# geduardo/SPARC

Hardware: AMD Instinct MI355X
Metric: env-steps/sec at batch 65536 (higher is better)
Workload: dtype f32 wire temperature + f64 scalar state

## Files before the change

### sparc_amd/csrc/wedm_common.h

```cpp
#pragma once


#ifndef WEDM_PACKED_DENSE
#define WEDM_PACKED_DENSE true
#endif
#ifndef WEDM_FUSED_DENSE
#define WEDM_FUSED_DENSE false
#endif
#ifndef WEDM_FUSED_MIN_BLOCKS
#define WEDM_FUSED_MIN_BLOCKS 2
#endif
#ifndef WEDM_PACKED_MIN_BLOCKS
#define WEDM_PACKED_MIN_BLOCKS 2
#endif
#ifndef WEDM_STREAM_PAIRED_LOADS
#define WEDM_STREAM_PAIRED_LOADS 1
#endif
#ifndef WEDM_STREAM_DENSE_QUIET
#define WEDM_STREAM_DENSE_QUIET 1
#endif
#ifndef WEDM_STREAM_REGWALK
#define WEDM_STREAM_REGWALK 1
#endif
#ifndef WEDM_PIN_STAGE
#define WEDM_PIN_STAGE 0
#endif
#ifndef WEDM_PREFETCH_N1
#define WEDM_PREFETCH_N1 0
#endif

#define WEDM_MAX_C 160
#define WEDM_MAX_TILES (WEDM_MAX_C / 8 + 1)
struct WalkTable {
    int32_t C;
    int32_t n_tiles;
    uint32_t zj[WEDM_MAX_TILES * 8];
    uint32_t iv[WEDM_MAX_TILES * 8];
    uint32_t kind[WEDM_MAX_TILES];
    uint32_t split[WEDM_MAX_TILES];
    uint32_t chunk_flags[16][4];
    uint32_t kind_n_mask, kind_s_mask;
    uint32_t split_pack[3];
    uint32_t kind_ne_mask, kind_nj_mask;
    uint32_t kind_n1_mask;
};
enum { TILE_N = 0, TILE_B = 1, TILE_S = 2 };

struct KArgs {
    Hot hot;
    Cold cold;
    int32_t num_envs;
    int32_t n_substeps;
    int32_t n_seg_max;
    const WalkTable* walk;
    int32_t trace_next;
    int32_t trace_slot;
    wedm_trace_desc trace;
    unsigned long long* dbg;
    int32_t* pulse;
    const double* envp;
    const double* wmat;
    double* sig;
};

__device__ __forceinline__ ColdRef kernarg_cold() {
    return ColdRef{(ColdPtr)((const WEDM_AS4 char*)__builtin_amdgcn_kernarg_segment_ptr() + offsetof(KArgs, cold))};
}

__device__ __forceinline__ PulseRef kernarg_pulse() {
    return PulseRef{(PulseSlot)((const WEDM_AS4 char*)__builtin_amdgcn_kernarg_segment_ptr() + offsetof(KArgs, pulse))};
}

__device__ __forceinline__ const double* wedm::kernarg_envp() {
    typedef const double* const WEDM_AS4* EnvpSlot;
    EnvpSlot p = (EnvpSlot)((const WEDM_AS4 char*)__builtin_amdgcn_kernarg_segment_ptr() + offsetof(KArgs, envp));
    asm volatile("" : "+s"(p));
    return *p;
}

__device__ __forceinline__ const double* wedm::kernarg_wmat() {
    typedef const double* const WEDM_AS4* WmatSlot;
    WmatSlot p = (WmatSlot)((const WEDM_AS4 char*)__builtin_amdgcn_kernarg_segment_ptr() + offsetof(KArgs, wmat));
    asm volatile("" : "+s"(p));
    return *p;
}

__device__ __forceinline__ SigRef kernarg_sig() {
    return SigRef{(SigSlot)((const WEDM_AS4 char*)__builtin_amdgcn_kernarg_segment_ptr() + offsetof(KArgs, sig))};
}

#include "wedm_lifecycle.h"

#define WEDM_TRACING(k) (TRACE && (k).trace_next < (k).n_substeps)
#define WEDM_TRACE_POINT(k, it, e, s, SCALAR_LANE, CELLS)                                        \
    if (TRACE && (it) == trace_next) {                                                           \
        const wedm_trace_desc& tr = (k).trace;                                                   \
        const int64_t tcol = trace_column(tr, (e));                                              \
        if (tcol >= 0) {                                                                         \
            if (SCALAR_LANE) trace_scalars(tr, tcol, (s), trace_slot, (k).hot.done_value == 0);  \
            if (tr.T) {                                                                          \
                const int64_t tcnt = tr.env_count;                                               \
                float* tT = tr.T + (int64_t)trace_slot * (k).n_seg_max * tcnt + tcol;            \
                CELLS;                                                                           \
            }                                                                                    \
        }                                                                                        \
        trace_next += tr.every;                                                                  \
        trace_slot = (trace_slot + 1 == tr.capacity) ? 0 : trace_slot + 1;                       \
    }

typedef float f4v __attribute__((ext_vector_type(4)));

struct GlobalT {
    float* base;
    int64_t qstride;
    __device__ __forceinline__ float ld(int i) const { return base[(int64_t)(i >> 2) * qstride + (i & 3)]; }
    __device__ __forceinline__ void st(int i, float v) const { base[(int64_t)(i >> 2) * qstride + (i & 3)] = v; }
    __device__ __forceinline__ f4v ldq(int q) const { return *(const f4v*)(base + (int64_t)q * qstride); }
    __device__ __forceinline__ void stq(int q, f4v v) const { *(f4v*)(base + (int64_t)q * qstride) = v; }
};
__device__ __forceinline__ GlobalT global_wire(float* T, int64_t stride, int64_t e) { return GlobalT{T + 4 * e, 4 * stride}; }

template <int L, bool TO_LDS, class Slot>
__device__ __forceinline__ void copy_wire(float* T, int64_t stride, int64_t e0, int num_envs, int n, int tid, float* lds, Slot slot) {
    constexpr int EPB = 256 / L;
    const int qr = tid / EPB, sel = tid % EPB;
    if (e0 + sel >= num_envs) return;
    float* const base = T + 4 * (e0 + sel);
    const int64_t qstride = 4 * stride;
    const int nq = (n + 3) >> 2;
    for (int q = qr; q < nq; q += L) {
        float* const g = base + (int64_t)q * qstride;
        if (TO_LDS) {
            const f4v v = *(const f4v*)g;
#pragma unroll
            for (int k = 0; k < 4; ++k)
                if (4 * q + k < n) lds[slot(4 * q + k) + sel * L] = v[k];
        } else if (4 * q + 3 < n) {
            f4v v;
#pragma unroll
            for (int k = 0; k < 4; ++k) v[k] = lds[slot(4 * q + k) + sel * L];
            *(f4v*)g = v;
        } else {
#pragma unroll
            for (int k = 0; k < 4; ++k)
                if (4 * q + k < n) g[k] = lds[slot(4 * q + k) + sel * L];
        }
    }
}

template <bool F64, class TA>
__device__ __forceinline__ float stencil_pass(const TA& T, const Geom& g, const Coef& c, const Persist& ps, const Hot& hot,
                                              const StencilF64& f64c, float h_base, float h_zone) {
    const float spool = hot.spool, tref = hot.tref, alpha = hot.alpha, tdiel = hot.tdiel;
    (void)tref; (void)alpha; (void)tdiel;
    const int n = g.n_seg;
    T.st(0, spool);
    float tmax = spool;
    if (n <= 1) return tmax;
    float tm1 = spool;
    float tc = T.ld(1);
    for (int i0 = 1; i0 < n; i0 += 8) {
        float nx[8];
#pragma unroll
        for (int u = 0; u < 8; ++u) {
            int idx = i0 + 1 + u;
            nx[u] = idx < n ? T.ld(idx) : 0.0f;
        }
#pragma unroll
        for (int u = 0; u < 8; ++u) {
            int i = i0 + u;
            if (i < n) {
                float tn;
                if (F64) tn = stencil_cell_f64(i, n, tm1, tc, nx[u], g, c, ps, f64c, h_base, h_zone);
                else tn = stencil_cell(i, n, tm1, tc, nx[u], g, c, ps, tref, alpha, tdiel);
                T.st(i, tn);
                tmax = tn > tmax ? tn : tmax;
                tm1 = tc;
                tc = nx[u];
            }
        }
    }
    return tmax;
}

template <uint32_t F, class TA>
__device__ __forceinline__ void run_substeps_h(const KArgs& k, const Hot& hot, const ColdRef cold, const Geom& g, int64_t e,
                                               uint32_t gid, Env& s, const TA& T, Sig& sg) {
    constexpr bool TRACE = (F & F_TRACE) != 0, F64 = (F & F_F64) != 0, PULSE = (F & F_PULSE) != 0;
    constexpr bool MAT = (F & F_MAT) != 0;
    Persist ps;
    init_persist<false, MAT>(hot, cold, e, s, ps);
    const StencilF64 f64c = stencil_f64_consts<F>(cold, e);
    const bool tracing = WEDM_TRACING(k);
    int trace_next = k.trace_next, trace_slot = k.trace_slot;
    (void)trace_next; (void)trace_slot;
    for (int it = 0; it < k.n_substeps; ++it) {
        if (!s.done) {
            const int32_t pk = PULSE ? pulse_kind(s) : 0;
            Coef c = scalar_prelude<F>(hot, cold, g, e, gid, s, ps, true);
            float tmax = s.broken ? s.tmax : stencil_pass<F64>(T, g, c, ps, hot, f64c, s.h_base, s.h_zone);
            env_step_done<F>(hot, cold, e, s, tmax, pk, true, sg);
        } else if (!tracing) {
            break;
        }
        WEDM_TRACE_POINT(k, it, e, s, true,
                         for (int i = 0; i < g.n_seg; ++i) tT[(int64_t)i * tcnt] = T.ld(i));
    }
}

template <uint32_t F, class TA>
__device__ __forceinline__ void run_substeps(const KArgs& k, const ColdRef cold, const Geom& g, int64_t e,
                                             uint32_t gid, Env& s, const TA& T, Sig& sg) {
    run_substeps_h<F, TA>(k, launch_hot<F>(k, cold, e, true), cold, g, e, gid, s, T, sg);
}

__device__ __forceinline__ float fmax_gt(float a, float b) { return __builtin_fmaxf(a, b); }

template <int CTRL>
__device__ __forceinline__ float dpp_lane_perm(float x) {
    return __int_as_float(__builtin_amdgcn_update_dpp(0, __float_as_int(x), CTRL, 0xF, 0xF, false));
}
template <int L>
__device__ __forceinline__ float max_over_env_lanes(float v) {
    static_assert(L == 1 || L == 2 || L == 4 || L == 8 || L == 16, "lanes per environment");
    if (L >= 2) v = fmax_gt(v, dpp_lane_perm<0xB1>(v));
    if (L >= 4) v = fmax_gt(v, dpp_lane_perm<0x4E>(v));
    if (L >= 8) v = fmax_gt(v, dpp_lane_perm<0x141>(v));
    if (L >= 16) v = fmax_gt(v, dpp_lane_perm<0x140>(v));
    return v;
}

#ifdef WEDM_STAMPS
#ifdef WEDM_STAMPS_REAL
#define WEDM_S2_CLOCK "s_memrealtime"
#else
#define WEDM_S2_CLOCK "s_memtime"
#endif
#define WEDM_S2_STAMP_DECL unsigned long long sst[12] = {0, 0, 0, 0, 0, 0, 0, 0, 0, 0, 0, 0}; \
    asm volatile(WEDM_S2_CLOCK " %0\n\ts_waitcnt lgkmcnt(0)" : "=s"(sst[7])::"memory")
#define WEDM_S2_STAMP(i) do { __builtin_amdgcn_sched_barrier(0); \
    asm volatile(WEDM_S2_CLOCK " %0\n\ts_waitcnt lgkmcnt(0)" : "=s"(sst[i])::"memory"); \
    __builtin_amdgcn_sched_barrier(0); } while (0)
#define WEDM_S2_STAMP_VM(i) do { __builtin_amdgcn_sched_barrier(0); \
    asm volatile("s_waitcnt vmcnt(0)\n\t" WEDM_S2_CLOCK " %0\n\ts_waitcnt lgkmcnt(0)" : "=s"(sst[i])::"memory"); \
    __builtin_amdgcn_sched_barrier(0); } while (0)
#define WEDM_S2_STAMP_OUT() do { if (k.dbg && (threadIdx.x & 63) == 0) { \
    unsigned long long* o = k.dbg + ((size_t)blockIdx.x * 4 + (threadIdx.x >> 6)) * 12; \
    for (int q = 0; q < 12; ++q) o[q] = sst[q]; } } while (0)
#else
#define WEDM_S2_STAMP_DECL do { } while (0)
#define WEDM_S2_STAMP(i) do { } while (0)
#define WEDM_S2_STAMP_VM(i) do { } while (0)
#define WEDM_S2_STAMP_OUT() do { } while (0)
#endif

typedef float f2 __attribute__((ext_vector_type(2)));

#define WEDM_STAGE_FENCE() __builtin_amdgcn_sched_barrier(0)
template <class V, bool JOULE, bool PERCELL, int W>
__device__ __forceinline__ void tile_staged(const V (&old)[10], V (&tn)[8], const int o, float k, float tuf,
                                            const V (&conv)[8], float tdiel, float adv, const V (&jfe)[8],
                                            float alpha, float tref) {
    V a[W], e[W], f[W], r[W];
#pragma unroll
    for (int u = 0; u < W; ++u) {
        a[u] = sub_twice(old[o + u], old[o + u + 1]);
        e[u] = old[o + u + 1] - tdiel;
        f[u] = old[o + u] - old[o + u + 1];
        if (JOULE) r[u] = old[o + u + 1] - tref;
    }
    WEDM_STAGE_FENCE();
#pragma unroll
    for (int u = 0; u < W; ++u) {
        e[u] = (PERCELL ? conv[o + u] : conv[0]) * e[u];
        f[u] = adv * f[u];
        if (JOULE) r[u] = alpha * r[u];
#if WEDM_PIN_STAGE
        asm volatile("" : "+v"(e[u]));
#endif
    }
    WEDM_STAGE_FENCE();
#pragma unroll
    for (int u = 0; u < W; ++u) {
        a[u] = a[u] + old[o + u + 2];
        if (JOULE) r[u] = 1.0f + r[u];
    }
    WEDM_STAGE_FENCE();
#pragma unroll
    for (int u = 0; u < W; ++u) {
        a[u] = k * a[u];
        if (JOULE) r[u] = (PERCELL ? jfe[o + u] : jfe[0]) * r[u];
    }
    WEDM_STAGE_FENCE();
    if (JOULE) {
#pragma unroll
        for (int u = 0; u < W; ++u) a[u] = a[u] + r[u];
        WEDM_STAGE_FENCE();
    }
#pragma unroll
    for (int u = 0; u < W; ++u) a[u] = a[u] - e[u];
    WEDM_STAGE_FENCE();
#pragma unroll
    for (int u = 0; u < W; ++u) a[u] = a[u] + f[u];
    WEDM_STAGE_FENCE();
#pragma unroll
    for (int u = 0; u < W; ++u) a[u] = a[u] * tuf;
    WEDM_STAGE_FENCE();
#pragma unroll
    for (int u = 0; u < W; ++u) tn[o + u] = old[o + u + 1] + a[u];
    WEDM_STAGE_FENCE();
}

#ifndef WEDM_STAGE_W
#define WEDM_STAGE_W 4
#endif
#ifndef WEDM_STAGE_W_PACKED
#define WEDM_STAGE_W_PACKED 2
#endif
template <class V, bool JOULE, bool PERCELL>
__device__ __forceinline__ void tile8_staged(const V (&old)[10], V (&tn)[8], float k, float tuf, const V (&conv)[8],
                                             float tdiel, float adv, const V (&jfe)[8], float alpha, float tref) {
    constexpr int W = sizeof(V) == 8 ? WEDM_STAGE_W_PACKED : WEDM_STAGE_W;
#pragma unroll
    for (int o = 0; o < 8; o += W)
        tile_staged<V, JOULE, PERCELL, W>(old, tn, o, k, tuf, conv, tdiel, adv, jfe, alpha, tref);
}

#ifndef WEDM_QUAD_STAGE_W
#define WEDM_QUAD_STAGE_W 2
#endif
template <bool JOULE, bool PERCELL, int W>
__device__ __forceinline__ void quad_stage_group(const f2 (&tm)[4], const f2 (&tc)[4], const f2 (&tp)[4], f2 (&tn)[4], const int o,
                                                 float k, float tuf, const f2 (&conv)[4], float tdiel, float adv,
                                                 const f2 (&jfe)[4], float alpha, float tref) {
    f2 a[W], e[W], f[W], r[W];
#pragma unroll
    for (int u = 0; u < W; ++u) {
        a[u] = sub_twice(tm[o + u], tc[o + u]);
        e[u] = tc[o + u] - tdiel;
        f[u] = tm[o + u] - tc[o + u];
        if (JOULE) r[u] = tc[o + u] - tref;
    }
    WEDM_STAGE_FENCE();
#pragma unroll
    for (int u = 0; u < W; ++u) {
        e[u] = (PERCELL ? conv[o + u] : conv[0]) * e[u];
        f[u] = adv * f[u];
        if (JOULE) r[u] = alpha * r[u];
    }
    WEDM_STAGE_FENCE();
#pragma unroll
    for (int u = 0; u < W; ++u) {
        a[u] = a[u] + tp[o + u];
        if (JOULE) r[u] = 1.0f + r[u];
    }
    WEDM_STAGE_FENCE();
#pragma unroll
    for (int u = 0; u < W; ++u) {
        a[u] = k * a[u];
        if (JOULE) r[u] = (PERCELL ? jfe[o + u] : jfe[0]) * r[u];
    }
    WEDM_STAGE_FENCE();
    if (JOULE) {
#pragma unroll
        for (int u = 0; u < W; ++u) a[u] = a[u] + r[u];
        WEDM_STAGE_FENCE();
    }
#pragma unroll
    for (int u = 0; u < W; ++u) a[u] = a[u] - e[u];
    WEDM_STAGE_FENCE();
#pragma unroll
    for (int u = 0; u < W; ++u) a[u] = a[u] + f[u];
    WEDM_STAGE_FENCE();
#pragma unroll
    for (int u = 0; u < W; ++u) a[u] = a[u] * tuf;
    WEDM_STAGE_FENCE();
#pragma unroll
    for (int u = 0; u < W; ++u) tn[o + u] = tc[o + u] + a[u];
    WEDM_STAGE_FENCE();
}
template <bool JOULE, bool PERCELL, int W = WEDM_QUAD_STAGE_W>
__device__ __forceinline__ void quad_staged(const f2 (&tm)[4], const f2 (&tc)[4], const f2 (&tp)[4], f2 (&tn)[4], float k,
                                            float tuf, const f2 (&conv)[4], float tdiel, float adv, const f2 (&jfe)[4],
                                            float alpha, float tref) {
#pragma unroll
    for (int o = 0; o < 4; o += W)
        quad_stage_group<JOULE, PERCELL, W>(tm, tc, tp, tn, o, k, tuf, conv, tdiel, adv, jfe, alpha, tref);
}

#ifndef WEDM_REGS_F64_FENCE
#define WEDM_REGS_F64_FENCE 1
#endif
template <bool JOULE>
__device__ __forceinline__ float cell_f64(float tm1, float tc, float tp1, double k64, double tuf64, double conv64, double tdiel64,
                                          double adv64, double jfe64, double alpha64, double tref64) {
    const double m = (double)tm1, t = (double)tc;
    float d = (float)(k64 * (__builtin_fma(-2.0, t, m) + (double)tp1));
    if (JOULE) {
        const double rho_T = 1.0 + alpha64 * (t - tref64);
        d = (float)((double)d + jfe64 * rho_T);
    }
    d = (float)((double)d - conv64 * (t - tdiel64));
    d = (float)((double)d + adv64 * (m - t));
    return (float)(t + (double)d * tuf64);
}

template <bool JOULE, bool PERCELL>
__device__ __forceinline__ void quad_f64(const f2 (&tm)[4], const f2 (&tc)[4], const f2 (&tp)[4], f2 (&tn)[4], const Geom& g,
                                         const f2 (&hc)[4], const Persist& ps, const f2 (&jfl)[4], const StencilF64& h, double jf64) {
    double cA = (double)hc[0].x * g.a64, cB = (double)hc[0].y * g.a64;
    double jA = (JOULE && jfl[0].x != 0.0f) ? jf64 : 0.0, jB = (JOULE && jfl[0].y != 0.0f) ? jf64 : 0.0;
#pragma unroll
    for (int u = 0; u < 4; ++u) {
        if (PERCELL && u > 0) {
            cA = (double)hc[u].x * g.a64; cB = (double)hc[u].y * g.a64;
            jA = (JOULE && jfl[u].x != 0.0f) ? jf64 : 0.0; jB = (JOULE && jfl[u].y != 0.0f) ? jf64 : 0.0;
        }
        tn[u].x = cell_f64<JOULE>(tm[u].x, tc[u].x, tp[u].x, g.k64, g.tuf64, cA, h.tdiel, ps.adv64, jA, h.alpha, h.tref);
#if WEDM_REGS_F64_FENCE < 0
        __builtin_amdgcn_sched_barrier(0);
#endif
        tn[u].y = cell_f64<JOULE>(tm[u].y, tc[u].y, tp[u].y, g.k64, g.tuf64, cB, h.tdiel, ps.adv64, jB, h.alpha, h.tref);
#if WEDM_REGS_F64_FENCE < 0
        __builtin_amdgcn_sched_barrier(0);
#elif WEDM_REGS_F64_FENCE > 0
        if ((u + 1) % WEDM_REGS_F64_FENCE == 0) __builtin_amdgcn_sched_barrier(0);
#endif
    }
}

template <bool F64, bool JOULE, bool PERCELL, int SW>
__device__ __forceinline__ void rw_quad(const f2 (&tm)[4], const f2 (&tc)[4], const f2 (&tp)[4], f2 (&tn)[4], const Geom& g,
                                        const f2 (&conv)[4], float tdiel, const Persist& ps, const f2 (&jfe)[4], float alpha,
                                        float tref, const StencilF64& h, const Coef& cf) {
    if (F64) quad_f64<JOULE, PERCELL>(tm, tc, tp, tn, g, conv, ps, jfe, h, cf.jf64);
    else quad_staged<JOULE, PERCELL, SW>(tm, tc, tp, tn, g.k, g.tuf, conv, tdiel, ps.adv, jfe, alpha, tref);
}
template <bool F64>
__device__ __forceinline__ float rw_cell(int i, int n_seg, float tm1, float tc, float tp1, const Geom& g, const Coef& cf,
                                         const Persist& ps, float tref, float alpha, float tdiel, const StencilF64& h,
                                         float h_base, float h_zone) {
    if (F64) return stencil_cell_f64(i, n_seg, tm1, tc, tp1, g, cf, ps, h, h_base, h_zone);
    return stencil_cell(i, n_seg, tm1, tc, tp1, g, cf, ps, tref, alpha, tdiel);
}

#define WEDM_REPORT_FROZEN(cond)                                                      \
    do {                                                                              \
        if (!kFrozenOk && __any(cond)) {                                              \
            int32_t* const seen = cold->frozen_seen;                                  \
            if (seen && (threadIdx.x & 63) == 0) *seen = 1;                           \
        }                                                                             \
    } while (0)

#ifdef WEDM_STAMPS
#define WEDM_STAMP(var)                                                      \
    do {                                                                     \
        __builtin_amdgcn_sched_barrier(0);                                   \
        asm volatile("s_memtime %0\n\ts_waitcnt lgkmcnt(0)" : "=s"(var)::"memory"); \
        __builtin_amdgcn_sched_barrier(0);                                   \
    } while (0)
#define WEDM_STAMP_DECL unsigned long long st0 = 0, st1 = 0, st2 = 0, st3 = 0, st4 = 0, acc0 = 0, acc1 = 0, acc2 = 0, acc3 = 0, tk0 = 0, tk1 = 0, accN = 0, accB = 0, accS = 0, cntN = 0, cntB = 0, cntS = 0
#define WEDM_STAMP_ACC() do { acc0 += st1 - st0; acc1 += st2 - st1; acc2 += st3 - st2; acc3 += st4 - st3; } while (0)
#define WEDM_STAMP_OUT()                                                                         \
    do {                                                                                         \
        if (k.dbg && (threadIdx.x & 63) == 0) {                                                  \
            unsigned long long* o = k.dbg + ((size_t)blockIdx.x * 4 + (threadIdx.x >> 6)) * 4;   \
            o[0] = acc0; o[1] = acc1; o[2] = acc2; o[3] = acc3;                                  \
            unsigned long long* o2 = k.dbg + (size_t)gridDim.x * 16 + ((size_t)blockIdx.x * 4 + (threadIdx.x >> 6)) * 6; \
            o2[0] = accN; o2[1] = accB; o2[2] = accS; o2[3] = cntN; o2[4] = cntB; o2[5] = cntS;  \
        }                                                                                        \
    } while (0)
#else
#define WEDM_STAMP(var) do { } while (0)
#define WEDM_STAMP_DECL do { } while (0)
#define WEDM_STAMP_ACC() do { } while (0)
#define WEDM_STAMP_OUT() do { } while (0)
#endif
```

### sparc_amd/csrc/wedm_k_regs.h

```cpp
#pragma once

struct cv4 {
    f2 v[4];
    __device__ __forceinline__ explicit cv4(f2 x) : v{x, x, x, x} {}
};

__device__ __forceinline__ float max3_raw(float a, float b, float c) {
    float r;
    asm("v_max3_f32 %0, %1, %2, %3" : "=v"(r) : "v"(a), "v"(b), "v"(c));
    return r;
}


#ifndef WEDM_REGS_DENSE
#define WEDM_REGS_DENSE WEDM_PACKED_DENSE
#endif
#ifndef WEDM_REGS_SW2
#define WEDM_REGS_SW2 2
#endif
#ifndef WEDM_REGS_PIN2
#define WEDM_REGS_PIN2 1
#endif
#ifndef WEDM_REGS_PAIR_SPLIT
#define WEDM_REGS_PAIR_SPLIT 1
#endif
template <int L, uint32_t F>
__global__ void __launch_bounds__(256, L) wedm_step_regs(const KArgs k) {
    static_assert((F & ~(F_TRACE | F_F64 | F_PULSE)) == 0, "forms of wedm_step_regs");
    constexpr bool TRACE = (F & F_TRACE) != 0, F64 = (F & F_F64) != 0, PULSE = (F & F_PULSE) != 0;
    constexpr int CELLS = 128;
    constexpr int H = CELLS / (2 * L);
    static_assert(L == 1 || L == 2, "one or two lanes per environment");
    static_assert(H % 8 == 0 && H / 8 <= 16, "whole tiles");
    constexpr int EPB = 256 / L;
    constexpr int SW = L == 1 ? 4 : WEDM_REGS_SW2;
    constexpr bool kF64 = F64;
    const ColdRef cold = kernarg_cold();
    Hot hv = k.hot;
    if (L == 1 || WEDM_REGS_PIN2 == 2) {
        pin_hot_in_vgprs(hv);
    } else if (WEDM_REGS_PIN2 == 1) {
        pin_mechanics_in_vgprs(hv);
        pin_quiet_in_vgprs(hv);
    }
    const int tid = threadIdx.x;
    const int c = tid % L;
    const int64_t e = (int64_t)blockIdx.x * EPB + tid / L;
    const bool live = e < k.num_envs;
    const bool writer = c == 0;
    const WalkTable* __restrict__ wt = k.walk;
    const int n = k.hot.n_seg;
    const int64_t stride = cold->s.stride;
    const int base = c * 2 * H;

    Env s;
    Geom g;
    Persist ps{0.0f, 0.0f, 0.0f, 0};
    load_geom(k.hot, cold, live ? e : 0, g);
    StencilF64 f64c{0.0, 0.0, 0.0};
    if (F64) {
        const wedm_params* pp = cold->p;
        f64c = StencilF64{pp->temp_ref, pp->alpha_rho, pp->dielectric_temperature};
        g.k64 = pp->k_cond; g.tuf64 = pp->tuf; g.a64 = pp->a_surf;
    }
    if (live) load_env(cold, e, s);
    else { s.done = WEDM_DEAD_LANE; s.unwind = 0.0; s.h_base = 0.0f; s.h_zone = 0.0f; }
    const int nq = (n + 3) >> 2;
    float* const Te = cold->s.T + (live ? e : 0) * 4;
    const int q0 = base / 4;
    f2 P[H];
#pragma unroll
    for (int q = 0; q < H / 4; ++q) {
        const f4v a = (q0 + q < nq) ? *(const f4v*)(Te + (int64_t)(q0 + q) * stride * 4) : f4v{0.0f, 0.0f, 0.0f, 0.0f};
        const f4v b = (q0 + H / 4 + q < nq) ? *(const f4v*)(Te + (int64_t)(q0 + H / 4 + q) * stride * 4) : f4v{0.0f, 0.0f, 0.0f, 0.0f};
#pragma unroll
        for (int u = 0; u < 4; ++u) P[4 * q + u] = f2{a[u], b[u]};
    }
    const float spool = k.hot.spool, tref = k.hot.tref, alpha = k.hot.alpha, tdiel = k.hot.tdiel;
    const bool reinit = live && s.done && WEDM_AUTORESET(cold);
    if (reinit) {
        reinit_env(cold, e, s, writer);
        pulse_reinit<PULSE>(kernarg_pulse(), cold, e, writer);
    }
    if (__any(reinit)) {
#pragma unroll
        for (int m = 0; m < H; ++m) P[m] = reinit ? f2{spool, spool} : P[m];
    }
    if (c == 0) P[0].x = spool;
    unfreeze_wire(k.hot, s);
    const bool frozen0 = s.done;
    if (!s.done) {
        s.ipk = peak_current(cold, s.mode, e);
        init_persist(k.hot, cold, e, s, ps);
    }
    const uint32_t gid = k.hot.env_id_offset + (uint32_t)e;

    const int n_tiles = wt->n_tiles;
    uint32_t zoneA = 0u, zoneB = 0u, jouleA = 0u, jouleB = 0u, joule_any = 0u;
    for (int t = 0; t < n_tiles; ++t) {
        const uint32_t lo = wt->zj[8 * t];
        zoneA |= ((lo >> (2 * c)) & 1u) << t;       zoneB |= ((lo >> (2 * c + 1)) & 1u) << t;
        jouleA |= ((lo >> (16 + 2 * c)) & 1u) << t; jouleB |= ((lo >> (17 + 2 * c)) & 1u) << t;
        joule_any |= ((lo >> 16) != 0u ? 1u : 0u) << t;
    }
    if (L == 1) {
        zoneA = __builtin_amdgcn_readfirstlane(zoneA); zoneB = __builtin_amdgcn_readfirstlane(zoneB);
        jouleA = __builtin_amdgcn_readfirstlane(jouleA); jouleB = __builtin_amdgcn_readfirstlane(jouleB);
    }
    joule_any = __builtin_amdgcn_readfirstlane(joule_any);
    const uint32_t kind_n = __builtin_amdgcn_readfirstlane(wt->kind_n_mask);
    const uint32_t kind_ne = __builtin_amdgcn_readfirstlane(wt->kind_ne_mask), kind_nj = __builtin_amdgcn_readfirstlane(wt->kind_nj_mask);
    const int last_base = (2 * L - 1) * H;
    const uint32_t last_tile = (n > last_base) ? (1u << ((n - 1 - last_base) >> 3)) : 0u;
    const bool owns_last = c == L - 1;

    f2 convp[H / 8];
    auto build_conv = [&]() {
        const float cz = F64 ? s.h_zone : ps.conv_zone, cb = F64 ? s.h_base : ps.conv_base;
#pragma unroll
        for (int t = 0; t < H / 8; ++t)
            convp[t] = f2{((zoneA >> t) & 1u) ? cz : cb, ((zoneB >> t) & 1u) ? cz : cb};
    };
    build_conv();
    const bool tracing = WEDM_TRACING(k);
    int trace_next = k.trace_next, trace_slot = k.trace_slot;
    (void)trace_next; (void)trace_slot;

    for (int it = 0; it < k.n_substeps; ++it) {
        if (__all(s.done) && !tracing) break;
        const int32_t pk = PULSE ? pulse_kind(s) : 0;
        Coef cf{0.0f, 0.0f, 0, -1};
        QuietTry qt;
        const bool was_quiet = quiet_prelude_t<WEDM_REGS_DENSE, 0u, L == 2 && WEDM_REGS_PAIR_SPLIT>(hv, cold, g, e, gid, s, qt, cf);
        if (!was_quiet) {
            if (!s.done) cf = scalar_prelude(hv, cold, g, e, gid, s, ps, writer, qt);
            build_conv();
        }
        freeze_wire(s);
        const bool act = !s.done;
        float tmax = spool;
        if (L == 1) asm volatile("" : "+s"(zoneA), "+s"(zoneB), "+s"(jouleA), "+s"(jouleB));
        else asm volatile("" : "+v"(zoneA), "+v"(zoneB), "+v"(jouleA), "+v"(jouleB));
        Geom gw = g;
        gw.n_seg = __builtin_amdgcn_readfirstlane(g.n_seg); gw.az_start = __builtin_amdgcn_readfirstlane(g.az_start);
        gw.az_end = __builtin_amdgcn_readfirstlane(g.az_end); gw.cb = __builtin_amdgcn_readfirstlane(g.cb);
        gw.ct = __builtin_amdgcn_readfirstlane(g.ct);
        asm volatile("" : "+s"(gw.n_seg), "+s"(gw.az_start), "+s"(gw.az_end), "+s"(gw.cb), "+s"(gw.ct));
        int nw = __builtin_amdgcn_readfirstlane(n);
        asm volatile("" : "+s"(nw));
        const float a_last = P[H - 1].x, b_first = P[0].y;
        float halo_l = spool, halo_r = 0.0f;
        if (L == 2) {
            const float give = c == 0 ? P[H - 1].y : P[0].x;
            const float got = __int_as_float(swap_with_neighbour(__float_as_int(give)));
            halo_l = c == 0 ? spool : got;
            halo_r = c == 0 ? got : 0.0f;
        }
        const float rw_h_base = s.h_base, rw_h_zone = s.h_zone;
#include "wedm_regs_walk.inc"
        if (L == 2) tmax = fmax_gt(tmax, __int_as_float(swap_with_neighbour(__float_as_int(tmax))));
        unfreeze_wire(hv, s);
        if (!s.done) {
            scalar_epilogue(hv, s, tmax);
            pulse_tally<PULSE>(kernarg_pulse(), cold, e, s, pk, writer);
            if (s.ctrl) control_step_outputs(cold, e, s, writer);
        }
        WEDM_TRACE_POINT(k, it, e, s, writer,
                         float* pa = tT + (int64_t)base * tcnt; float* pb = pa + (int64_t)H * tcnt;
                         int na = n - base; int nb = na - H;
                         asm volatile("" : "+v"(na), "+v"(nb));
                         _Pragma("unroll") for (int m = 0; m < H; ++m) {
                             if (m < na) *pa = P[m].x;
                             if (m < nb) *pb = P[m].y;
                             pa += tcnt; pb += tcnt;
                             asm volatile("" : "+v"(pa), "+v"(pb));
                         });
    }

    if (live) {
#pragma unroll
        for (int q = 0; q < 2 * H / 4; ++q) {
            const int m = (q % (H / 4)) * 4;
            const bool hi = q >= H / 4;
            const f4v w = hi ? f4v{P[m].y, P[m + 1].y, P[m + 2].y, P[m + 3].y} : f4v{P[m].x, P[m + 1].x, P[m + 2].x, P[m + 3].x};
            const int cell = base + 4 * q;
            if (cell + 3 < n) {
                *(f4v*)(Te + (int64_t)(q0 + q) * stride * 4) = w;
            } else {
#pragma unroll
                for (int u = 0; u < 4; ++u)
                    if (cell + u < n) Te[(int64_t)(q0 + q) * stride * 4 + u] = w[u];
            }
        }
    }
    if (live && writer) {
        if (WEDM_REWARD_ON(cold)) {
            if (!frozen0) write_reward(cold, e, s);
            else cold->s.reward[e] = 0.0f;
        }
        store_time_hi(cold, e, s, (uint32_t)k.n_substeps * (uint32_t)k.hot.dt_us);
        store_env(cold, e, s);
    }
}


__device__ __forceinline__ float dpp_row_shr1(float old, float x) {
    return __int_as_float(__builtin_amdgcn_update_dpp(__float_as_int(old), __float_as_int(x), 0x111, 0xF, 0xF, false));
}
__device__ __forceinline__ float dpp_row_shl1(float old, float x) {
    return __int_as_float(__builtin_amdgcn_update_dpp(__float_as_int(old), __float_as_int(x), 0x101, 0xF, 0xF, false));
}
template <int CTRL>
__device__ __forceinline__ float dpp_perm(float x) {
    return __int_as_float(__builtin_amdgcn_update_dpp(0, __float_as_int(x), CTRL, 0xF, 0xF, false));
}

#ifndef WEDM_WIDE_MIN_BLOCKS
#define WEDM_WIDE_MIN_BLOCKS 1
#endif

#ifndef WEDM_WIDE_SW
#define WEDM_WIDE_SW 2
#endif
#ifndef WEDM_WIDE_DENSE
#define WEDM_WIDE_DENSE WEDM_REGS_DENSE
#endif
#ifndef WEDM_WIDE_AUTO_MAX_LANES
#define WEDM_WIDE_AUTO_MAX_LANES 65536
#endif
constexpr int wide_min_blocks(uint32_t F) { return !(F & F_F64) ? WEDM_WIDE_MIN_BLOCKS : (F & F_MINB2) ? 2 : 1; }
template <int L, uint32_t F>
__global__ void __launch_bounds__(256, wide_min_blocks(F)) wedm_step_regs_wide(const KArgs k) {
    static_assert((F & ~(F_CUT | F_TRACE | F_F64 | F_MINB2 | F_PULSE)) == 0 && (!(F & F_MINB2) || (F & F_F64)),
                  "forms of wedm_step_regs_wide");
    constexpr bool CUT = (F & F_CUT) != 0, TRACE = (F & F_TRACE) != 0, F64 = (F & F_F64) != 0, PULSE = (F & F_PULSE) != 0;
    constexpr int H = 16, MINB = wide_min_blocks(F);
    static_assert(H % 8 == 0 && H <= 32, "whole tiles");
    static_assert(L == 4 || L == 8 || L == 16, "the lanes of an environment lie in one DPP row");
    constexpr int EPB = 256 / L;
    constexpr int SW = WEDM_WIDE_SW;
    const ColdRef cold = kernarg_cold();
    Hot hv = k.hot;
    if (MINB == 1) pin_hot_in_vgprs(hv);
    const int tid = threadIdx.x;
    const int c = tid % L;
    const int64_t e = (int64_t)blockIdx.x * EPB + tid / L;
    const bool live = e < k.num_envs;
    const bool writer = c == 0;
    const int n = k.hot.n_seg;
    const int64_t stride = cold->s.stride;
    const int base = c * 2 * H;

    Env s;
    Geom g;
    Persist ps{0.0f, 0.0f, 0.0f, 0};
    load_geom(k.hot, cold, live ? e : 0, g);
    StencilF64 f64c{0.0, 0.0, 0.0};
    if (F64) {
        const wedm_params* pp = cold->p;
        f64c = StencilF64{pp->temp_ref, pp->alpha_rho, pp->dielectric_temperature};
        g.k64 = pp->k_cond; g.tuf64 = pp->tuf; g.a64 = pp->a_surf;
    }
    if (live) load_env(cold, e, s);
    else { s.done = WEDM_DEAD_LANE; s.unwind = 0.0; s.h_base = 0.0f; s.h_zone = 0.0f; }
    const int nq = (n + 3) >> 2;
    float* const Te = cold->s.T + (live ? e : 0) * 4;
    const int q0 = base / 4;
    f2 P[H];
#pragma unroll
    for (int q = 0; q < H / 4; ++q) {
        const f4v a = (q0 + q < nq) ? *(const f4v*)(Te + (int64_t)(q0 + q) * stride * 4) : f4v{0.0f, 0.0f, 0.0f, 0.0f};
        const f4v b = (q0 + H / 4 + q < nq) ? *(const f4v*)(Te + (int64_t)(q0 + H / 4 + q) * stride * 4) : f4v{0.0f, 0.0f, 0.0f, 0.0f};
#pragma unroll
        for (int u = 0; u < 4; ++u) P[4 * q + u] = f2{a[u], b[u]};
    }
    const float spool = k.hot.spool, tref = k.hot.tref, alpha = k.hot.alpha, tdiel = k.hot.tdiel;
    const bool reinit = live && s.done && WEDM_AUTORESET(cold);
    if (reinit) {
        reinit_env(cold, e, s, writer);
        pulse_reinit<PULSE>(kernarg_pulse(), cold, e, writer);
    }
    if (__any(reinit)) {
#pragma unroll
        for (int m = 0; m < H; ++m) P[m] = reinit ? f2{spool, spool} : P[m];
    }
    if (c == 0) P[0].x = spool;
    unfreeze_wire(k.hot, s);
    const bool frozen0 = s.done;
    if (!s.done) {
        s.ipk = peak_current(cold, s.mode, e);
        init_persist(k.hot, cold, e, s, ps);
    }
    const uint32_t gid = k.hot.env_id_offset + (uint32_t)e;

    const int nA = min(max(n - base, 0), H), nB = min(max(n - base - H, 0), H);
    uint32_t zoneA = 0u, zoneB = 0u, jouleA = 0u, jouleB = 0u;
#pragma unroll
    for (int m = 0; m < H; ++m) {
        const int ia = base + m, ib = base + H + m;
        zoneA |= (ia >= g.az_start && ia < g.az_end) ? (1u << m) : 0u;
        zoneB |= (ib >= g.az_start && ib < g.az_end) ? (1u << m) : 0u;
        jouleA |= (ia >= g.cb && ia <= g.ct) ? (1u << m) : 0u;
        jouleB |= (ib >= g.cb && ib <= g.ct) ? (1u << m) : 0u;
    }
    uint32_t cut = 0u;
    if (CUT) {
#pragma unroll
        for (int t = 0; t < H / 8; ++t)
            cut |= __any((nA > 8 * t && nA < 8 * t + 8) || (nB > 8 * t && nB < 8 * t + 8)) ? (1u << t) : 0u;
        cut = __builtin_amdgcn_readfirstlane(cut);
    }
    const int ll = n - 1 - base;
    const bool owns_last = ll >= 0 && ll < 2 * H;
    const int lloc = (n - 1) & (2 * H - 1);
    const bool last_in_b = lloc >= H;
    const uint32_t last_tile = ((n & 7) == 0) ? (1u << ((lloc & (H - 1)) >> 3)) : 0u;
    f2 jm[H], convc[H];
#pragma unroll
    for (int m = 0; m < H; ++m) jm[m] = f2{((jouleA >> m) & 1u) ? 1.0f : 0.0f, ((jouleB >> m) & 1u) ? 1.0f : 0.0f};
    auto build_conv = [&]() {
        const float cz = F64 ? s.h_zone : ps.conv_zone, cb = F64 ? s.h_base : ps.conv_base;
#pragma unroll
        for (int m = 0; m < H; ++m)
            convc[m] = f2{((zoneA >> m) & 1u) ? cz : cb, ((zoneB >> m) & 1u) ? cz : cb};
    };
    build_conv();
    WEDM_STAMP_DECL;
    const bool tracing = WEDM_TRACING(k);
    int trace_next = k.trace_next, trace_slot = k.trace_slot;
    (void)trace_next; (void)trace_slot;

    for (int it = 0; it < k.n_substeps; ++it) {
        if (__all(s.done) && !tracing) break;
        WEDM_STAMP(st0);
        const int32_t pk = PULSE ? pulse_kind(s) : 0;
        Coef cf{0.0f, 0.0f, 0, -1};
        QuietTry qt;
        const bool was_quiet = quiet_prelude_t<WEDM_WIDE_DENSE>(hv, cold, g, e, gid, s, qt, cf);
        if (!was_quiet) {
            if (!s.done) cf = scalar_prelude(hv, cold, g, e, gid, s, ps, writer, qt);
            build_conv();
        }
        freeze_wire(s);
        WEDM_STAMP(st1);
        const bool act = !s.done;
        float tmax = spool;
        const float a_last = P[H - 1].x, b_first = P[0].y;
        float halo_l = dpp_row_shr1(spool, P[H - 1].y), halo_r = dpp_row_shl1(0.0f, P[0].x);
        if (L < 16) { halo_l = c == 0 ? spool : halo_l; halo_r = c == L - 1 ? 0.0f : halo_r; }
        const bool busy = __any(cf.joule_on != 0 || cf.pidx >= 0 || cf.q != 0.0f);
        auto walk = [&](auto plain_tag) {
            constexpr bool PLAIN = decltype(plain_tag)::value;
            const Coef cz{0.0f, 0.0f, 0, -1};
            const Coef& cw = PLAIN ? cz : cf;
            Geom gw = g;
            int nw = n;
            auto prep_gw = [&]() {
                gw.n_seg = __builtin_amdgcn_readfirstlane(g.n_seg); gw.az_start = __builtin_amdgcn_readfirstlane(g.az_start);
                gw.az_end = __builtin_amdgcn_readfirstlane(g.az_end); gw.cb = __builtin_amdgcn_readfirstlane(g.cb);
                gw.ct = __builtin_amdgcn_readfirstlane(g.ct);
                asm volatile("" : "+s"(gw.n_seg), "+s"(gw.az_start), "+s"(gw.az_end), "+s"(gw.cb), "+s"(gw.ct));
                nw = __builtin_amdgcn_readfirstlane(n);
                asm volatile("" : "+s"(nw));
            };
            if (!PLAIN) prep_gw();
            const float jf_lane = (!PLAIN && cf.joule_on) ? (F64 ? 1.0f : cf.jf) : 0.0f;
            const bool joule_wave = !PLAIN && __any(jf_lane != 0.0f);
            const int pcell = (!PLAIN && cf.pidx >= 1 && cf.pidx >= base && cf.pidx < base + 2 * H) ? cf.pidx - base : -1;
            uint32_t ptiles = 0u;
            if (!PLAIN && __any(pcell >= 0)) {
                const int pt = pcell >= 0 ? ((pcell & (H - 1)) >> 3) : -1;
#pragma unroll
                for (int t = 0; t < H / 8; ++t) ptiles |= __any(pt == t) ? (1u << t) : 0u;
            }
            const uint32_t odd = ptiles | last_tile | cut;
            const f2 jfp = f2{jf_lane, jf_lane};
            f2 leftp = f2{halo_l, a_last};
#pragma unroll
            for (int t = 0; t < H / 8; ++t) {
                const int j = 8 * t;
                f2 tm[8], tc[8], tp[8], pn[8];
#pragma unroll
                for (int u = 0; u < 8; ++u) {
                    tc[u] = P[j + u];
                    tm[u] = u == 0 ? leftp : P[j + u - 1];
                    tp[u] = (j + u + 1 < H) ? P[j + u + 1 < H ? j + u + 1 : 0] : f2{b_first, halo_r};
                }
                leftp = tc[7];
                {
                    f2 tmA[4], tcA[4], tpA[4], pnA[4], tmB[4], tcB[4], tpB[4], pnB[4], cvA[4], cvB[4];
#pragma unroll
                    for (int u = 0; u < 4; ++u) {
                        tmA[u] = tm[u]; tcA[u] = tc[u]; tpA[u] = tp[u]; tmB[u] = tm[4 + u]; tcB[u] = tc[4 + u]; tpB[u] = tp[4 + u];
                        cvA[u] = convc[j + u]; cvB[u] = convc[j + 4 + u];
                    }
                    if (!PLAIN && joule_wave) {
                        f2 jvA[4], jvB[4];
#pragma unroll
                        for (int u = 0; u < 4; ++u) { jvA[u] = jm[j + u] * jfp; jvB[u] = jm[j + 4 + u] * jfp; }
                        rw_quad<F64, true, true, SW>(tmA, tcA, tpA, pnA, g, cvA, tdiel, ps, jvA, alpha, tref, f64c, cf);
                        rw_quad<F64, true, true, SW>(tmB, tcB, tpB, pnB, g, cvB, tdiel, ps, jvB, alpha, tref, f64c, cf);
                    } else {
                        rw_quad<F64, false, true, SW>(tmA, tcA, tpA, pnA, g, cvA, tdiel, ps, cvA, alpha, tref, f64c, cw);
                        rw_quad<F64, false, true, SW>(tmB, tcB, tpB, pnB, g, cvB, tdiel, ps, cvB, alpha, tref, f64c, cw);
                    }
#pragma unroll
                    for (int u = 0; u < 4; ++u) { pn[u] = pnA[u]; pn[4 + u] = pnB[u]; }
                    if (t == 0) pn[0].x = (c == 0) ? spool : pn[0].x;
                    if ((odd >> t) & 1u) {
                        if (PLAIN) prep_gw();
                        if ((last_tile >> t) & 1u) {
                            const float x = rw_cell<F64>(base + (last_in_b ? H : 0) + j + 7, nw, last_in_b ? tm[7].y : tm[7].x,
                                                         last_in_b ? tc[7].y : tc[7].x, 0.0f, gw, cw, ps, tref, alpha, tdiel, f64c, s.h_base, s.h_zone);
                            const bool hx = owns_last && !last_in_b, hy = owns_last && last_in_b;
                            pn[7].x = hx ? x : pn[7].x; pn[7].y = hy ? x : pn[7].y;
                        }
                        if ((cut >> t) & 1u) {
                            int lw = lloc;
                            asm volatile("" : "+s"(lw));
#pragma unroll
                            for (int u = 0; u < 8; ++u) {
                                if (lw == j + u) {
                                    const float x = rw_cell<F64>(base + j + u, nw, tm[u].x, tc[u].x, 0.0f, gw, cw, ps, tref, alpha, tdiel, f64c, s.h_base, s.h_zone);
                                    pn[u].x = owns_last ? x : pn[u].x;
                                }
                                if (lw == H + j + u) {
                                    const float x = rw_cell<F64>(base + H + j + u, nw, tm[u].y, tc[u].y, 0.0f, gw, cw, ps, tref, alpha, tdiel, f64c, s.h_base, s.h_zone);
                                    pn[u].y = owns_last ? x : pn[u].y;
                                }
                            }
                        }
                        if (!PLAIN && ((ptiles >> t) & 1u)) {
#pragma unroll
                            for (int u = 0; u < 8; ++u) {
                                if (__any(pcell == j + u)) {
                                    const float x = rw_cell<F64>(base + j + u, nw, (base + j + u == 1) ? spool : tm[u].x, tc[u].x, tp[u].x, gw, cf, ps, tref, alpha, tdiel, f64c, s.h_base, s.h_zone);
                                    pn[u].x = (pcell == j + u) ? x : pn[u].x;
                                }
                                if (__any(pcell == H + j + u)) {
                                    const float x = rw_cell<F64>(base + H + j + u, nw, tm[u].y, tc[u].y, tp[u].y, gw, cf, ps, tref, alpha, tdiel, f64c, s.h_base, s.h_zone);
                                    pn[u].y = (pcell == H + j + u) ? x : pn[u].y;
                                }
                            }
                        }
                    }
                    float mx, my;
                    if ((cut >> t) & 1u) {
                        mx = spool; my = spool;
                        int va = nA, vb = nB;
                        asm volatile("" : "+v"(va), "+v"(vb));
#pragma unroll
                        for (int u = 0; u < 8; ++u) {
                            mx = (j + u < va) ? fmax_gt(mx, pn[u].x) : mx;
                            my = (j + u < vb) ? fmax_gt(my, pn[u].y) : my;
                        }
                    } else {
                        mx = max3_raw(pn[0].x, pn[1].x, pn[2].x); my = max3_raw(pn[0].y, pn[1].y, pn[2].y);
                        mx = max3_raw(mx, pn[3].x, pn[4].x); my = max3_raw(my, pn[3].y, pn[4].y);
                        mx = max3_raw(mx, pn[5].x, pn[6].x); my = max3_raw(my, pn[5].y, pn[6].y);
                        mx = fmax_gt(mx, pn[7].x); my = fmax_gt(my, pn[7].y);
                        mx = nA > j ? mx : spool; my = nB > j ? my : spool;
                    }
                    tmax = max3_raw(tmax, mx, my);
                }
#pragma unroll
                for (int u = 0; u < 8; ++u) P[j + u] = pn[u];
            }
        };
        if (act) {
            if (busy) walk(std::false_type{});
            else walk(std::true_type{});
        }
        WEDM_STAMP(st2);
        tmax = fmax_gt(tmax, dpp_perm<0xB1>(tmax));
        tmax = fmax_gt(tmax, dpp_perm<0x4E>(tmax));
        if (L >= 8) tmax = fmax_gt(tmax, dpp_perm<0x141>(tmax));
        if (L >= 16) tmax = fmax_gt(tmax, dpp_perm<0x140>(tmax));
        unfreeze_wire(hv, s);
        WEDM_STAMP(st3);
        if (!s.done) {
            scalar_epilogue(hv, s, tmax);
            pulse_tally<PULSE>(kernarg_pulse(), cold, e, s, pk, writer);
            if (s.ctrl) control_step_outputs(cold, e, s, writer);
        }
        WEDM_STAMP(st4);
        WEDM_STAMP_ACC();
        WEDM_TRACE_POINT(k, it, e, s, writer,
                         for (int m = 0; m < H; ++m) {
                             if (base + m < n) tT[(int64_t)(base + m) * tcnt] = P[m].x;
                             if (base + H + m < n) tT[(int64_t)(base + H + m) * tcnt] = P[m].y;
                         });
    }
    WEDM_STAMP_OUT();

    if (live) {
#pragma unroll
        for (int q = 0; q < 2 * H / 4; ++q) {
            const int m = (q % (H / 4)) * 4;
            const bool hi = q >= H / 4;
            const f4v w = hi ? f4v{P[m].y, P[m + 1].y, P[m + 2].y, P[m + 3].y} : f4v{P[m].x, P[m + 1].x, P[m + 2].x, P[m + 3].x};
            const int cell = base + 4 * q;
            if (cell + 3 < n) {
                *(f4v*)(Te + (int64_t)(q0 + q) * stride * 4) = w;
            } else {
#pragma unroll
                for (int u = 0; u < 4; ++u)
                    if (cell + u < n) Te[(int64_t)(q0 + q) * stride * 4 + u] = w[u];
            }
        }
    }
    if (live && writer) {
        if (WEDM_REWARD_ON(cold)) {
            if (!frozen0) write_reward(cold, e, s);
            else cold->s.reward[e] = 0.0f;
        }
        store_time_hi(cold, e, s, (uint32_t)k.n_substeps * (uint32_t)k.hot.dt_us);
        store_env(cold, e, s);
    }
}
```

### sparc_amd/csrc/wedm_regs_walk.inc

```
        if (act) {
            const bool all_slow = __any(cf.q < 0.0f);
            const float jf_lane = cf.joule_on ? (kF64 ? 1.0f : cf.jf) : 0.0f;
            const bool joule_wave = __any(jf_lane != 0.0f);
            const uint32_t n_now = all_slow ? 0u : (kind_n | kind_ne | (joule_wave ? 0u : kind_nj));
            const int pcell = (cf.pidx >= 1 && cf.pidx >= base && cf.pidx < base + 2 * H) ? cf.pidx - base : -1;
            uint32_t ptiles = 0u;
            if (__any(pcell >= 0)) {
                const int pt = pcell >= 0 ? ((pcell & (H - 1)) >> 3) : -1;
#pragma unroll
                for (int t = 0; t < H / 8; ++t) ptiles |= __any(pt == t) ? (1u << t) : 0u;
            }
            const uint32_t general = ~n_now | (joule_wave ? joule_any : 0u) | ptiles | last_tile;
            f2 leftp = f2{halo_l, a_last};
#pragma unroll
            for (int t = 0; t < H / 8; ++t) {
                if (t < n_tiles) {
                    const int j = 8 * t;
                    f2 tm[8], tc[8], tp[8], pn[8];
#pragma unroll
                    for (int u = 0; u < 8; ++u) {
                        tc[u] = P[j + u];
                        tm[u] = u == 0 ? leftp : P[j + u - 1];
                        tp[u] = (j + u + 1 < H) ? P[j + u + 1 < H ? j + u + 1 : 0] : f2{b_first, halo_r};
                    }
                    leftp = tc[7];
                    f2 cv[4], jv[4];
                    cv[0] = convp[t];
                    f2 tmA[4], tcA[4], tpA[4], pnA[4], tmB[4], tcB[4], tpB[4], pnB[4];
#pragma unroll
                    for (int u = 0; u < 4; ++u) { tmA[u] = tm[u]; tcA[u] = tc[u]; tpA[u] = tp[u]; tmB[u] = tm[4 + u]; tcB[u] = tc[4 + u]; tpB[u] = tp[4 + u]; }
                    if (!((general >> t) & 1u)) {
                        jv[0] = f2{0.0f, 0.0f};
                        rw_quad<kF64, false, false, SW>(tmA, tcA, tpA, pnA, g, cv, tdiel, ps, jv, alpha, tref, f64c, cf);
                        rw_quad<kF64, false, false, SW>(tmB, tcB, tpB, pnB, g, cv, tdiel, ps, jv, alpha, tref, f64c, cf);
#pragma unroll
                        for (int u = 0; u < 4; ++u) { pn[u] = pnA[u]; pn[4 + u] = pnB[u]; }
                        if (t == 0) pn[0].x = (c == 0) ? spool : pn[0].x;
                        float m0 = max3_raw(tmax, pn[0].x, pn[0].y), m1 = max3_raw(pn[1].x, pn[1].y, pn[2].x);
                        m0 = max3_raw(m0, pn[2].y, pn[3].x); m1 = max3_raw(m1, pn[3].y, pn[4].x);
                        m0 = max3_raw(m0, pn[4].y, pn[5].x); m1 = max3_raw(m1, pn[5].y, pn[6].x);
                        m0 = max3_raw(m0, pn[6].y, pn[7].x);
                        tmax = max3_raw(m0, m1, pn[7].y);
                    } else if (((n_now | (all_slow ? 0u : kind_nj)) >> t) & 1u) {
                        jv[0] = f2{((jouleA >> t) & 1u) ? jf_lane : 0.0f, ((jouleB >> t) & 1u) ? jf_lane : 0.0f};
                        if (!((n_now >> t) & 1u)) {
                            f2 jq[8];
#pragma unroll
                            for (int u = 0; u < 8; ++u) {
                                const uint32_t zj = wt->zj[j + u];
                                jq[u] = f2{((zj >> (16 + 2 * c)) & 1u) ? jf_lane : 0.0f, ((zj >> (17 + 2 * c)) & 1u) ? jf_lane : 0.0f};
                            }
                            f2 jvA[4], jvB[4];
#pragma unroll
                            for (int u = 0; u < 4; ++u) { jvA[u] = jq[u]; jvB[u] = jq[4 + u]; }
                            rw_quad<kF64, true, true, SW>(tmA, tcA, tpA, pnA, g, cv4(cv[0]).v, tdiel, ps, jvA, alpha, tref, f64c, cf);
                            rw_quad<kF64, true, true, SW>(tmB, tcB, tpB, pnB, g, cv4(cv[0]).v, tdiel, ps, jvB, alpha, tref, f64c, cf);
                        } else if (joule_wave && ((joule_any >> t) & 1u)) {
                            rw_quad<kF64, true, false, SW>(tmA, tcA, tpA, pnA, g, cv, tdiel, ps, jv, alpha, tref, f64c, cf);
                            rw_quad<kF64, true, false, SW>(tmB, tcB, tpB, pnB, g, cv, tdiel, ps, jv, alpha, tref, f64c, cf);
                        } else {
                            rw_quad<kF64, false, false, SW>(tmA, tcA, tpA, pnA, g, cv, tdiel, ps, jv, alpha, tref, f64c, cf);
                            rw_quad<kF64, false, false, SW>(tmB, tcB, tpB, pnB, g, cv, tdiel, ps, jv, alpha, tref, f64c, cf);
                        }
#pragma unroll
                        for (int u = 0; u < 4; ++u) { pn[u] = pnA[u]; pn[4 + u] = pnB[u]; }
                        if (t == 0) pn[0].x = (c == 0) ? spool : pn[0].x;
                        const bool has_last = ((last_tile >> t) & 1u) && owns_last;
                        float m0 = max3_raw(tmax, pn[0].x, pn[0].y), m1 = max3_raw(pn[1].x, pn[1].y, pn[2].x);
                        m0 = max3_raw(m0, pn[2].y, pn[3].x); m1 = max3_raw(m1, pn[3].y, pn[4].x);
                        m0 = max3_raw(m0, pn[4].y, pn[5].x); m1 = max3_raw(m1, pn[5].y, pn[6].x);
                        m0 = max3_raw(m0, pn[6].y, pn[7].x);
                        tmax = max3_raw(m0, m1, has_last ? spool : pn[7].y);
                        if ((last_tile >> t) & 1u) {
                            const float x = rw_cell<kF64>(base + H + j + 7, nw, tm[7].y, tc[7].y, 0.0f, gw, cf, ps, tref, alpha, tdiel, f64c, rw_h_base, rw_h_zone);
                            pn[7].y = has_last ? x : pn[7].y;
                            tmax = has_last ? fmax_gt(tmax, x) : tmax;
                        }
                        if ((ptiles >> t) & 1u) {
#pragma unroll
                            for (int u = 0; u < 8; ++u) {
                                if (__any(pcell == j + u)) {
                                    const float x = rw_cell<kF64>(base + j + u, nw, (base + j + u == 1) ? spool : tm[u].x, tc[u].x, tp[u].x, gw, cf, ps, tref, alpha, tdiel, f64c, rw_h_base, rw_h_zone);
                                    pn[u].x = (pcell == j + u) ? x : pn[u].x;
                                    tmax = (pcell == j + u) ? fmax_gt(tmax, x) : tmax;
                                }
                                if (__any(pcell == H + j + u)) {
                                    const float x = rw_cell<kF64>(base + H + j + u, nw, tm[u].y, tc[u].y, tp[u].y, gw, cf, ps, tref, alpha, tdiel, f64c, rw_h_base, rw_h_zone);
                                    pn[u].y = (pcell == H + j + u) ? x : pn[u].y;
                                    tmax = (pcell == H + j + u) ? fmax_gt(tmax, x) : tmax;
                                }
                            }
                        }
                    } else {
#pragma unroll
                        for (int u = 0; u < 8; ++u) {
                            pn[u] = tc[u];
                            const int ia = base + j + u, ib = base + H + j + u;
                            {
                                const float x = (ia >= 1) ? rw_cell<kF64>(ia, nw, (ia == 1) ? spool : tm[u].x, tc[u].x, tp[u].x, gw, cf, ps, tref, alpha, tdiel, f64c, rw_h_base, rw_h_zone) : spool;
                                pn[u].x = ia < nw ? x : pn[u].x;
                                tmax = ia < nw ? fmax_gt(tmax, x) : tmax;
                            }
                            {
                                const float x = rw_cell<kF64>(ib, nw, tm[u].y, tc[u].y, tp[u].y, gw, cf, ps, tref, alpha, tdiel, f64c, rw_h_base, rw_h_zone);
                                pn[u].y = ib < nw ? x : pn[u].y;
                                tmax = ib < nw ? fmax_gt(tmax, x) : tmax;
                            }
                        }
                    }
#pragma unroll
                    for (int u = 0; u < 8; ++u) P[j + u] = pn[u];
#ifdef WEDM_REGS_WALK_TILE_FENCE
                    __builtin_amdgcn_sched_barrier(0);
#endif
                }
            }
        }
```

Baseline: 16.46 billion.

## Pack tile masks, recompute env index, add plain-step fast path in walk

Packs the four per-lane zone/joule tile bitmasks into one 32-bit word and recomputes the environment index from the wave base and lane id instead of keeping it live across the substep loop, both to cut register pressure. The walk also gains a wave-uniform fast path: when no lane in the wave has joule heating, a pulse cell or nonzero charge, it skips the per-lane coefficient checks and uses precomputed scalar tile masks. Optional timing stamps split quiet and non-quiet steps for profiling. The extra packing and unpacking adds ALU work, and the fast-path branch adds a wave vote every substep.

```diff
diff --git a/sparc_amd/csrc/wedm_common.h b/sparc_amd/csrc/wedm_common.h
--- a/sparc_amd/csrc/wedm_common.h
+++ b/sparc_amd/csrc/wedm_common.h
@@ -461,6 +461,11 @@
     } while (0)
 #define WEDM_STAMP_DECL unsigned long long st0 = 0, st1 = 0, st2 = 0, st3 = 0, st4 = 0, acc0 = 0, acc1 = 0, acc2 = 0, acc3 = 0, tk0 = 0, tk1 = 0, accN = 0, accB = 0, accS = 0, cntN = 0, cntB = 0, cntS = 0
 #define WEDM_STAMP_ACC() do { acc0 += st1 - st0; acc1 += st2 - st1; acc2 += st3 - st2; acc3 += st4 - st3; } while (0)
+#define WEDM_STAMP_ACC_SPLIT(quiet)                                                             \
+    do {                                                                                        \
+        if (quiet) { WEDM_STAMP_ACC(); ++cntS; }                                                \
+        else { accN += st1 - st0; accB += st2 - st1; accS += st4 - st2; ++cntN; }               \
+    } while (0)
 #define WEDM_STAMP_OUT()                                                                         \
     do {                                                                                         \
         if (k.dbg && (threadIdx.x & 63) == 0) {                                                  \
@@ -474,5 +479,6 @@
 #define WEDM_STAMP(var) do { } while (0)
 #define WEDM_STAMP_DECL do { } while (0)
 #define WEDM_STAMP_ACC() do { } while (0)
+#define WEDM_STAMP_ACC_SPLIT(quiet) do { } while (0)
 #define WEDM_STAMP_OUT() do { } while (0)
 #endif
diff --git a/sparc_amd/csrc/wedm_k_regs.h b/sparc_amd/csrc/wedm_k_regs.h
--- a/sparc_amd/csrc/wedm_k_regs.h
+++ b/sparc_amd/csrc/wedm_k_regs.h
@@ -45,7 +45,14 @@
     }
     const int tid = threadIdx.x;
     const int c = tid % L;
-    const int64_t e = (int64_t)blockIdx.x * EPB + tid / L;
+    int64_t e = (int64_t)blockIdx.x * EPB + tid / L;
+    const uint32_t wave_env0 = __builtin_amdgcn_readfirstlane((uint32_t)e);
+    auto env_index = [&]() -> int64_t {
+        uint32_t all = ~0u;
+        asm volatile("" : "+s"(all));
+        const uint32_t lane = __builtin_amdgcn_mbcnt_hi(all, __builtin_amdgcn_mbcnt_lo(all, 0u));
+        return (int64_t)(wave_env0 + lane / L);
+    };
     const bool live = e < k.num_envs;
     const bool writer = c == 0;
     const WalkTable* __restrict__ wt = k.walk;
@@ -66,7 +73,7 @@
     if (live) load_env(cold, e, s);
     else { s.done = WEDM_DEAD_LANE; s.unwind = 0.0; s.h_base = 0.0f; s.h_zone = 0.0f; }
     const int nq = (n + 3) >> 2;
-    float* const Te = cold->s.T + (live ? e : 0) * 4;
+    float* Te = cold->s.T + (live ? e : 0) * 4;
     const int q0 = base / 4;
     f2 P[H];
 #pragma unroll
@@ -93,20 +100,17 @@
         s.ipk = peak_current(cold, s.mode, e);
         init_persist(k.hot, cold, e, s, ps);
     }
-    const uint32_t gid = k.hot.env_id_offset + (uint32_t)e;
-
+
+    static_assert(H / 8 <= 8, "tile flags: a byte per mask");
     const int n_tiles = wt->n_tiles;
-    uint32_t zoneA = 0u, zoneB = 0u, jouleA = 0u, jouleB = 0u, joule_any = 0u;
+    uint32_t tile_flags = 0u, joule_any = 0u;
     for (int t = 0; t < n_tiles; ++t) {
         const uint32_t lo = wt->zj[8 * t];
-        zoneA |= ((lo >> (2 * c)) & 1u) << t;       zoneB |= ((lo >> (2 * c + 1)) & 1u) << t;
-        jouleA |= ((lo >> (16 + 2 * c)) & 1u) << t; jouleB |= ((lo >> (17 + 2 * c)) & 1u) << t;
+        tile_flags |= (((lo >> (2 * c)) & 1u) << t) | (((lo >> (2 * c + 1)) & 1u) << (8 + t));
+        tile_flags |= (((lo >> (16 + 2 * c)) & 1u) << (16 + t)) | (((lo >> (17 + 2 * c)) & 1u) << (24 + t));
         joule_any |= ((lo >> 16) != 0u ? 1u : 0u) << t;
     }
-    if (L == 1) {
-        zoneA = __builtin_amdgcn_readfirstlane(zoneA); zoneB = __builtin_amdgcn_readfirstlane(zoneB);
-        jouleA = __builtin_amdgcn_readfirstlane(jouleA); jouleB = __builtin_amdgcn_readfirstlane(jouleB);
-    }
+    if (L == 1) tile_flags = __builtin_amdgcn_readfirstlane(tile_flags);
     joule_any = __builtin_amdgcn_readfirstlane(joule_any);
     const uint32_t kind_n = __builtin_amdgcn_readfirstlane(wt->kind_n_mask);
     const uint32_t kind_ne = __builtin_amdgcn_readfirstlane(wt->kind_ne_mask), kind_nj = __builtin_amdgcn_readfirstlane(wt->kind_nj_mask);
@@ -116,18 +120,23 @@
 
     f2 convp[H / 8];
     auto build_conv = [&]() {
+        const uint32_t zoneA = tile_flags & 0xFFu, zoneB = (tile_flags >> 8) & 0xFFu;
         const float cz = F64 ? s.h_zone : ps.conv_zone, cb = F64 ? s.h_base : ps.conv_base;
 #pragma unroll
         for (int t = 0; t < H / 8; ++t)
             convp[t] = f2{((zoneA >> t) & 1u) ? cz : cb, ((zoneB >> t) & 1u) ? cz : cb};
     };
     build_conv();
+    WEDM_STAMP_DECL;
     const bool tracing = WEDM_TRACING(k);
     int trace_next = k.trace_next, trace_slot = k.trace_slot;
     (void)trace_next; (void)trace_slot;
 
     for (int it = 0; it < k.n_substeps; ++it) {
         if (__all(s.done) && !tracing) break;
+        WEDM_STAMP(st0);
+        e = env_index();
+        const uint32_t gid = k.hot.env_id_offset + (uint32_t)e;
         const int32_t pk = PULSE ? pulse_kind(s) : 0;
         Coef cf{0.0f, 0.0f, 0, -1};
         QuietTry qt;
@@ -137,10 +146,12 @@
             build_conv();
         }
         freeze_wire(s);
+        WEDM_STAMP(st1);
         const bool act = !s.done;
         float tmax = spool;
-        if (L == 1) asm volatile("" : "+s"(zoneA), "+s"(zoneB), "+s"(jouleA), "+s"(jouleB));
-        else asm volatile("" : "+v"(zoneA), "+v"(zoneB), "+v"(jouleA), "+v"(jouleB));
+        if (L == 1) asm volatile("" : "+s"(tile_flags));
+        else asm volatile("" : "+v"(tile_flags));
+        const uint32_t jouleA = (tile_flags >> 16) & 0xFFu, jouleB = tile_flags >> 24;
         Geom gw = g;
         gw.n_seg = __builtin_amdgcn_readfirstlane(g.n_seg); gw.az_start = __builtin_amdgcn_readfirstlane(g.az_start);
         gw.az_end = __builtin_amdgcn_readfirstlane(g.az_end); gw.cb = __builtin_amdgcn_readfirstlane(g.cb);
@@ -158,13 +169,17 @@
         }
         const float rw_h_base = s.h_base, rw_h_zone = s.h_zone;
 #include "wedm_regs_walk.inc"
+        WEDM_STAMP(st2);
         if (L == 2) tmax = fmax_gt(tmax, __int_as_float(swap_with_neighbour(__float_as_int(tmax))));
         unfreeze_wire(hv, s);
+        WEDM_STAMP(st3);
         if (!s.done) {
             scalar_epilogue(hv, s, tmax);
             pulse_tally<PULSE>(kernarg_pulse(), cold, e, s, pk, writer);
             if (s.ctrl) control_step_outputs(cold, e, s, writer);
         }
+        WEDM_STAMP(st4);
+        WEDM_STAMP_ACC_SPLIT(was_quiet);
         WEDM_TRACE_POINT(k, it, e, s, writer,
                          float* pa = tT + (int64_t)base * tcnt; float* pb = pa + (int64_t)H * tcnt;
                          int na = n - base; int nb = na - H;
@@ -176,7 +191,10 @@
                              asm volatile("" : "+v"(pa), "+v"(pb));
                          });
     }
-
+    WEDM_STAMP_OUT();
+
+    e = env_index();
+    Te = cold->s.T + (live ? e : 0) * 4;
     if (live) {
 #pragma unroll
         for (int q = 0; q < 2 * H / 4; ++q) {
diff --git a/sparc_amd/csrc/wedm_regs_walk.inc b/sparc_amd/csrc/wedm_regs_walk.inc
--- a/sparc_amd/csrc/wedm_regs_walk.inc
+++ b/sparc_amd/csrc/wedm_regs_walk.inc
@@ -1,16 +1,27 @@
         if (act) {
-            const bool all_slow = __any(cf.q < 0.0f);
-            const float jf_lane = cf.joule_on ? (kF64 ? 1.0f : cf.jf) : 0.0f;
-            const bool joule_wave = __any(jf_lane != 0.0f);
-            const uint32_t n_now = all_slow ? 0u : (kind_n | kind_ne | (joule_wave ? 0u : kind_nj));
-            const int pcell = (cf.pidx >= 1 && cf.pidx >= base && cf.pidx < base + 2 * H) ? cf.pidx - base : -1;
+            uint32_t n_now = __builtin_amdgcn_readfirstlane(kind_n | kind_ne | kind_nj);
+            uint32_t general = __builtin_amdgcn_readfirstlane(~(kind_n | kind_ne | kind_nj) | last_tile);
+            asm volatile("" : "+s"(n_now), "+s"(general));
+            bool all_slow = false, joule_wave = false;
+            float jf_lane = 0.0f;
+            int pcell = -1;
             uint32_t ptiles = 0u;
-            if (__any(pcell >= 0)) {
-                const int pt = pcell >= 0 ? ((pcell & (H - 1)) >> 3) : -1;
+#ifndef WEDM_REGS_WALK_NO_PLAIN
+            if (__any(cf.joule_on != 0 || cf.pidx >= 0 || cf.q != 0.0f))
+#endif
+            {
+                all_slow = __any(cf.q < 0.0f);
+                jf_lane = cf.joule_on ? (kF64 ? 1.0f : cf.jf) : 0.0f;
+                joule_wave = __any(jf_lane != 0.0f);
+                n_now = all_slow ? 0u : (kind_n | kind_ne | (joule_wave ? 0u : kind_nj));
+                pcell = (cf.pidx >= 1 && cf.pidx >= base && cf.pidx < base + 2 * H) ? cf.pidx - base : -1;
+                if (__any(pcell >= 0)) {
+                    const int pt = pcell >= 0 ? ((pcell & (H - 1)) >> 3) : -1;
 #pragma unroll
-                for (int t = 0; t < H / 8; ++t) ptiles |= __any(pt == t) ? (1u << t) : 0u;
+                    for (int t = 0; t < H / 8; ++t) ptiles |= __any(pt == t) ? (1u << t) : 0u;
+                }
+                general = ~n_now | (joule_wave ? joule_any : 0u) | ptiles | last_tile;
             }
-            const uint32_t general = ~n_now | (joule_wave ? joule_any : 0u) | ptiles | last_tile;
             f2 leftp = f2{halo_l, a_last};
 #pragma unroll
             for (int t = 0; t < H / 8; ++t) {
```

Result: faster. 16.84 billion (median of 6 runs) (+2.3%).
